# zakuro-ai/asr

Measured on AMD Instinct MI355X. Metric: utterances/sec (10 s, 161-bin) DS2 5x1024 BiGRU CTC train step, higher is better.
Workload: dtype bf16

## Files before the change

### asr_amd/csrc/conv_bf16.hip

```cpp
#include "common.h"
#include <stdlib.h>

namespace {

typedef __bf16 bf16x8 __attribute__((ext_vector_type(8)));

constexpr int TT = 128, KT = 11, PT = 5, CH = 32;
constexpr int NPIX = TT + KT - 1;
constexpr int IPITCH = 80;
constexpr int WROW = KT * 2 * 2 * 32 * 16;

__device__ __attribute__((aligned(16))) float g_zero_cb[4] = {0.f, 0.f, 0.f, 0.f};

struct CArgs {
  const __bf16* in;
  const __bf16* wpk;
  const float* bias;
  float* out;
  const int* lens;
  int B, Din, T, Dtot, KD, SD, PD, OS, OO;
  int gx, gy, gz;
};

constexpr int IN_CHUNKS = NPIX * 4;
constexpr int IN_IT = (IN_CHUNKS + 255) / 256;
constexpr int W_CHUNKS = WROW / 16;
constexpr int W_IT = (W_CHUNKS + 255) / 256;

template <int SD, int R>
__global__ __launch_bounds__(256) void conv2_bf16_rows_kernel(CArgs a, int n_out, float* __restrict__ stat_part) {
  constexpr int RING = (R - 1) * SD + 1;
  constexpr int SLOT = NPIX * IPITCH;
  __shared__ __attribute__((aligned(16))) char in_lds[RING * SLOT];
  __shared__ __attribute__((aligned(16))) char w_lds[WROW];
  const int tid = threadIdx.x, lane = tid & 63, wave = tid >> 6;
  const int half = lane >> 5, l31 = lane & 31;
  int bx, by, bz;
  {
    const int total = a.gx * a.gy * a.gz, id = blockIdx.x;
    const int lin = (total & 7) == 0 ? (id & 7) * (total >> 3) + (id >> 3) : id;
    by = lin % a.gy;
    const int pair = lin / a.gy;
    bx = pair % a.gx; bz = pair / a.gx;
  }
  const int t0 = bx * TT, o0 = R * by, b = bz;
  const int len = a.lens ? min(a.lens[b], a.T) : a.T;
  const int t = t0 + wave * 32 + l31;
  auto out_ptr = [&](int o, int co) { return a.out + (((long long)b * CH + co) * a.Dtot + (a.OS * o + a.OO)) * a.T + t; };
  if (t0 >= len) {
    if (t < a.T) {
#pragma unroll
      for (int q = 0; q < R; ++q)
        if (o0 + q < n_out) {
#pragma unroll
          for (int r = 0; r < 16; ++r) *out_ptr(o0 + q, (r & 3) + 8 * (r >> 2) + 4 * half) = 0.f;
        }
    }
    return;
  }
  f32x16 acc[R];
#pragma unroll
  for (int q = 0; q < R; ++q)
#pragma unroll
    for (int r = 0; r < 16; ++r) acc[q][r] = 0.f;

  const int f0 = SD * o0 - a.PD;
  f32x4 ri[IN_IT], rw[W_IT];
  auto load_in = [&](int f) {
    const bool rowok = f >= 0 && f < a.Din;
    const char* rowp = reinterpret_cast<const char*>(a.in + (((long long)b * a.Din + (rowok ? f : 0)) * a.T) * CH);
#pragma unroll
    for (int u = 0; u < IN_IT; ++u) {
      const int c = tid + 256 * u;
      const int pix = c >> 2, q = c & 3;
      const int tt = t0 - PT + pix;
      const bool ok = rowok && c < IN_CHUNKS && tt >= 0 && tt < a.T;
      const void* p = ok ? (const void*)(rowp + ((long long)tt * CH) * 2 + q * 16) : (const void*)g_zero_cb;
      ri[u] = *reinterpret_cast<const f32x4*>(p);
    }
  };
  auto store_in = [&](int slot) {
#pragma unroll
    for (int u = 0; u < IN_IT; ++u) {
      const int c = tid + 256 * u;
      if (c < IN_CHUNKS) *reinterpret_cast<f32x4*>(in_lds + slot * SLOT + (c >> 2) * IPITCH + (c & 3) * 16) = ri[u];
    }
  };
  auto load_w = [&](int kd) {
    const char* wp = reinterpret_cast<const char*>(a.wpk) + (long long)kd * WROW;
#pragma unroll
    for (int u = 0; u < W_IT; ++u) {
      const int c = tid + 256 * u;
      rw[u] = *reinterpret_cast<const f32x4*>(wp + (c < W_CHUNKS ? c : 0) * 16);
    }
  };
  auto store_w = [&]() {
#pragma unroll
    for (int u = 0; u < W_IT; ++u) {
      const int c = tid + 256 * u;
      if (c < W_CHUNKS) *reinterpret_cast<f32x4*>(w_lds + c * 16) = rw[u];
    }
  };
#pragma unroll
  for (int j = 0; j < RING - 1; ++j) {
    load_in(f0 + j);
    store_in(j);
  }
  load_in(f0 + RING - 1);
  load_w(0);
  const int pix_off = (wave * 32 + l31) * IPITCH + half * 16;
  const char* abase = w_lds + half * (32 * 16) + l31 * 16;
  int slot0 = 0;
  for (int kd = 0; kd < a.KD; ++kd) {
    __syncthreads();
    {
      int snew = slot0 + RING - 1;
      if (snew >= RING) snew -= RING;
      store_in(snew);
    }
    store_w();
    __syncthreads();
    if (kd + 1 < a.KD) {
      load_in(f0 + kd + RING);
      load_w(kd + 1);
    }
    const char* bq[R];
#pragma unroll
    for (int q = 0; q < R; ++q) {
      int sl = slot0 + q * SD;
      if (sl >= RING) sl -= RING;
      bq[q] = in_lds + sl * SLOT + pix_off;
    }
#pragma unroll
    for (int kt = 0; kt < KT; ++kt) {
#pragma unroll
      for (int kk = 0; kk < 2; ++kk) {
        const bf16x8 af = *reinterpret_cast<const bf16x8*>(abase + (kt * 2 + kk) * (2 * 32 * 16));
#pragma unroll
        for (int q = 0; q < R; ++q) {
          const bf16x8 x = *reinterpret_cast<const bf16x8*>(bq[q] + kt * IPITCH + kk * 32);
          acc[q] = __builtin_amdgcn_mfma_f32_32x32x16_bf16(af, x, acc[q], 0, 0, 0);
        }
      }
    }
    slot0 = slot0 + 1 == RING ? 0 : slot0 + 1;
  }
  float bv[16];
#pragma unroll
  for (int r = 0; r < 16; ++r) bv[r] = a.bias ? a.bias[(r & 3) + 8 * (r >> 2) + 4 * half] : 0.f;
  float s1[16], s2[16];
#pragma unroll
  for (int r = 0; r < 16; ++r) { s1[r] = 0.f; s2[r] = 0.f; }
#pragma unroll
  for (int q = 0; q < R; ++q)
    if (o0 + q < n_out) {
#pragma unroll
      for (int r = 0; r < 16; ++r) {
        const float v = (t >= len || t >= a.T) ? 0.f : acc[q][r] + bv[r];
        if (t < a.T) *out_ptr(o0 + q, (r & 3) + 8 * (r >> 2) + 4 * half) = v;
        s1[r] += v;
        s2[r] += v * v;
      }
    }
  if (stat_part) {
    __shared__ float red[4][32][2];
#pragma unroll
    for (int r = 0; r < 16; ++r) {
#pragma unroll
      for (int m = 1; m < 32; m <<= 1) { s1[r] += __shfl_xor(s1[r], m); s2[r] += __shfl_xor(s2[r], m); }
      if (l31 == 0) { const int co = (r & 3) + 8 * (r >> 2) + 4 * half; red[wave][co][0] = s1[r]; red[wave][co][1] = s2[r]; }
    }
    __syncthreads();
    if (tid < 64) {
      const int co = tid >> 1, w = tid & 1;
      const float sum = ((red[0][co][w] + red[1][co][w]) + red[2][co][w]) + red[3][co][w];
      const long long blk = ((long long)bz * a.gy + by) * a.gx + bx;
      stat_part[(blk * 32 + co) * 2 + w] = sum;
    }
  }
}

__global__ __launch_bounds__(256) void nhwc_cast_kernel(const float* __restrict__ src, __bf16* __restrict__ dst, int Bn, int D, int T) {
  __shared__ float tile[CH][65];
  const int t0 = blockIdx.x * 64, d = blockIdx.y, b = blockIdx.z;
  const int tx = threadIdx.x & 63, ty = threadIdx.x >> 6;
#pragma unroll
  for (int i = 0; i < 8; ++i) {
    const int c = ty + 4 * i, t = t0 + tx;
    tile[c][tx] = (t < T) ? src[(((long long)b * CH + c) * D + d) * T + t] : 0.f;
  }
  __syncthreads();
  const int c = threadIdx.x & 31, tq = threadIdx.x >> 5;
#pragma unroll
  for (int i = 0; i < 8; ++i) {
    const int tl = tq + 8 * i, t = t0 + tl;
    if (t < T) dst[(((long long)b * D + d) * T + t) * CH + c] = (__bf16)tile[c][tl];
  }
}

__global__ void pack_conv2_bf16_kernel(const float* __restrict__ W, __bf16* __restrict__ wf, __bf16* __restrict__ wd0, __bf16* __restrict__ wd1) {
  const int per_row = WROW / 2;
  const int nf = 21 * per_row, n0 = 11 * per_row, n1 = 10 * per_row;
  const int idx = blockIdx.x * blockDim.x + threadIdx.x;
  if (idx >= nf + n0 + n1) return;
  int which, i;
  if (idx < nf) { which = 0; i = idx; } else if (idx < nf + n0) { which = 1; i = idx - nf; } else { which = 2; i = idx - nf - n0; }
  const int j = i & 7, m = (i >> 3) & 31, kg = (i >> 8) & 1, kk = (i >> 9) & 1;
  const int rest = i >> 10;
  const int kt = rest % KT, kdr = rest / KT;
  const int kch = kk * 16 + kg * 8 + j;
  float v;
  if (which == 0) {
    v = W[((m * 32 + kch) * 21 + kdr) * 11 + kt];
    wf[i] = (__bf16)v;
  } else {
    const int p = which - 1, KDe = (21 - p + 1) / 2;
    v = W[((kch * 32 + m) * 21 + (2 * (KDe - 1 - kdr) + p)) * 11 + (10 - kt)];
    (which == 1 ? wd0 : wd1)[i] = (__bf16)v;
  }
}

}

extern "C" size_t ds2_conv2_bf16_packed_bytes(int which) { return (size_t)(which == 0 ? 21 : which == 1 ? 11 : 10) * WROW; }

extern "C" int ds2_conv2_pack_bf16(const float* w2, void* wf, void* wd0, void* wd1, void* stream) {
  DS2_REQUIRE(w2 && wf && wd0 && wd1, "ds2_conv2_pack_bf16: null pointer");
  const int total = (21 + 11 + 10) * (WROW / 2);
  hipLaunchKernelGGL(pack_conv2_bf16_kernel, dim3(ceil_div(total, 256)), dim3(256), 0, (hipStream_t)stream, w2, (__bf16*)wf, (__bf16*)wd0,
                     (__bf16*)wd1);
  DS2_LAUNCH_CHECK("pack_conv2_bf16_kernel");
  return 0;
}

extern "C" int ds2_nhwc_bf16_f32(const float* src, void* dst, int B, int D, int T, void* stream) {
  DS2_REQUIRE(src && dst && B > 0 && D > 0 && T > 0, "ds2_nhwc_bf16_f32: bad args");
  hipLaunchKernelGGL(nhwc_cast_kernel, dim3(ceil_div(T, 64), D, B), dim3(256), 0, (hipStream_t)stream, src, (__bf16*)dst, B, D, T);
  DS2_LAUNCH_CHECK("nhwc_cast_kernel");
  return 0;
}

extern "C" int ds2_conv2_fwd_bf16_stat_blocks(int B, int D1, int T) {
  const int D2 = (D1 + 2 * 10 - 21) / 2 + 1;
  return ceil_div(T, TT) * ceil_div(D2, 3) * B;
}

extern "C" int ds2_conv2_fwd_bf16_stats(const void* a1_nhwc, const void* wf, const float* bias, const int* lens_dev, float* y2, int B, int D1,
                                        int T, float* stat_part, void* stream) {
  DS2_REQUIRE(a1_nhwc && wf && y2, "ds2_conv2_fwd_bf16: null pointer");
  const int D2 = (D1 + 2 * 10 - 21) / 2 + 1;
  CArgs a{};
  a.in = (const __bf16*)a1_nhwc; a.wpk = (const __bf16*)wf; a.bias = bias; a.out = y2; a.lens = lens_dev;
  a.B = B; a.Din = D1; a.T = T; a.Dtot = D2; a.KD = 21; a.SD = 2; a.PD = 10; a.OS = 1; a.OO = 0;
  if (stat_part) DS2_HIP(hipMemsetAsync(stat_part, 0, (size_t)ds2_conv2_fwd_bf16_stat_blocks(B, D1, T) * 64 * sizeof(float), (hipStream_t)stream));
  a.gx = ceil_div(T, TT); a.gy = ceil_div(D2, 3); a.gz = B;
  hipLaunchKernelGGL((conv2_bf16_rows_kernel<2, 3>), dim3(a.gx * a.gy * a.gz), dim3(256), 0, (hipStream_t)stream, a, D2, stat_part);
  DS2_LAUNCH_CHECK("conv2_bf16_rows_kernel fwd");
  return 0;
}

extern "C" int ds2_conv2_fwd_bf16(const void* a1_nhwc, const void* wf, const float* bias, const int* lens_dev, float* y2, int B, int D1,
                                  int T, void* stream) {
  return ds2_conv2_fwd_bf16_stats(a1_nhwc, wf, bias, lens_dev, y2, B, D1, T, nullptr, stream);
}

extern "C" int ds2_conv2_dgrad_bf16(const void* dy2_nhwc, const void* wd0, const void* wd1, float* da1, int B, int D1, int T, void* stream) {
  DS2_REQUIRE(dy2_nhwc && wd0 && wd1 && da1, "ds2_conv2_dgrad_bf16: null pointer");
  const int D2 = (D1 + 2 * 10 - 21) / 2 + 1;
  for (int p = 0; p < 2; ++p) {
    const int KDe = (21 - p + 1) / 2;
    const int n_o = (D1 - p + 1) / 2;
    CArgs a{};
    a.in = (const __bf16*)dy2_nhwc; a.wpk = (const __bf16*)(p == 0 ? wd0 : wd1); a.bias = nullptr; a.out = da1; a.lens = nullptr;
    a.B = B; a.Din = D2; a.T = T; a.Dtot = D1; a.KD = KDe; a.SD = 1; a.PD = KDe - 6; a.OS = 2; a.OO = p;
    a.gx = ceil_div(T, TT); a.gy = ceil_div(n_o, 4); a.gz = B;
    hipLaunchKernelGGL((conv2_bf16_rows_kernel<1, 4>), dim3(a.gx * a.gy * a.gz), dim3(256), 0, (hipStream_t)stream, a, n_o, (float*)nullptr);
  }
  DS2_LAUNCH_CHECK("conv2_bf16_rows_kernel dgrad");
  return 0;
}

namespace {

constexpr int WT = 64;
constexpr int WK = WT + 16;
constexpr int WPITCH = 176;
constexpr int KDG = 3;
constexpr int TAPS = KDG * KT;
constexpr int TPW = (TAPS + 3) / 4;

struct WArgs {
  const __bf16* a1p;
  const __bf16* dyp;
  float* part;
  const int* lens;
  int B, D1, D2, T, Tp, pairs_per_chunk;
};

typedef unsigned int u32x4 __attribute__((ext_vector_type(4)));

__device__ __forceinline__ void store_shifted_copies(const u32x4 lo, const u32x4 hi, char* dst ) {
  const unsigned W[8] = {lo.x, lo.y, lo.z, lo.w, hi.x, hi.y, hi.z, hi.w};
#pragma unroll
  for (int r = 0; r < 8; ++r) {
    const int w0 = (8 - r) >> 1;
    u32x4 o;
    if ((r & 1) == 0) {
      o = u32x4{W[w0], W[w0 + 1], W[w0 + 2], W[w0 + 3]};
    } else {
      o = u32x4{__builtin_amdgcn_alignbit(W[w0 + 1], W[w0], 16), __builtin_amdgcn_alignbit(W[w0 + 2], W[w0 + 1], 16),
                __builtin_amdgcn_alignbit(W[w0 + 3], W[w0 + 2], 16), __builtin_amdgcn_alignbit(W[w0 + 4], W[w0 + 3], 16)};
    }
    *reinterpret_cast<u32x4*>(dst + r * 32 * WPITCH) = o;
  }
}

__global__ __launch_bounds__(256) __attribute__((amdgpu_waves_per_eu(2, 2))) void conv2_wgrad_bf16_kernel(WArgs a) {
  __shared__ __attribute__((aligned(16))) char dy_lds[8 * 32 * WPITCH];
  __shared__ __attribute__((aligned(16))) char a1_lds[KDG * 32 * WPITCH];
  const int tid = threadIdx.x, lane = tid & 63;
  const int wave = __builtin_amdgcn_readfirstlane(tid >> 6);
  const int l31 = lane & 31, half = lane >> 5;
  const int grp = blockIdx.x, chunk = blockIdx.y;
  const int kd0 = grp * KDG;

  f32x16 acc[TPW];
#pragma unroll
  for (int i = 0; i < TPW; ++i)
#pragma unroll
    for (int r = 0; r < 16; ++r) acc[i][r] = 0.f;

  constexpr int NDY = 2, NA1 = (KDG * 32 * 10 + 255) / 256;
  u32x4 dlo[NDY], dhi[NDY], av[NA1];

  const int npairs = a.B * a.D2;
  const int pend = min(npairs, (chunk + 1) * a.pairs_per_chunk);
  int p = chunk * a.pairs_per_chunk, t0 = 0, len = 0;
  auto settle = [&]() {
    while (p < pend) {
      len = a.lens ? min(a.lens[p / a.D2], a.T) : a.T;
      if (t0 < len) return true;
      ++p;
      t0 = 0;
    }
    return false;
  };
  auto load_tile = [&]() {
    const int b = p / a.D2, o = p % a.D2;
#pragma unroll
    for (int k = 0; k < NDY; ++k) {
      const int idx = tid + 256 * k;
      const int co = idx / 11, m = idx % 11;
      const __bf16* row = a.dyp + (((long long)b * 32 + min(co, 31)) * a.D2 + o) * a.Tp;
      const int xl = t0 - 8 + m * 8, xh = xl + 8;
      const bool okl = idx < 352 && m >= 2 && m < 2 + WT / 8 && xl + 8 <= a.Tp;
      const bool okh = idx < 352 && m + 1 >= 2 && m + 1 < 2 + WT / 8 && xh + 8 <= a.Tp;
      dlo[k] = *reinterpret_cast<const u32x4*>(okl ? (const void*)(row + xl) : (const void*)g_zero_cb);
      dhi[k] = *reinterpret_cast<const u32x4*>(okh ? (const void*)(row + xh) : (const void*)g_zero_cb);
    }
#pragma unroll
    for (int k = 0; k < NA1; ++k) {
      const int c = tid + 256 * k;
      const int ch = c % 10, ci = (c / 10) % 32, kdl = c / 320;
      const int f = 2 * o + (kd0 + kdl) - 10;
      const int x0 = t0 + ch * 8;
      const bool ok = c < KDG * 320 && (kd0 + kdl) < 21 && f >= 0 && f < a.D1 && x0 + 8 <= a.Tp;
      av[k] = *reinterpret_cast<const u32x4*>(ok ? (const void*)(a.a1p + (((long long)b * 32 + ci) * a.D1 + f) * a.Tp + x0)
                                                 : (const void*)g_zero_cb);
    }
  };

  bool have = settle();
  if (have) load_tile();
  while (have) {
    __syncthreads();
#pragma unroll
    for (int k = 0; k < NDY; ++k) {
      const int idx = tid + 256 * k;
      if (idx < 352) store_shifted_copies(dlo[k], dhi[k], dy_lds + (idx / 11) * WPITCH + (idx % 11) * 16);
    }
#pragma unroll
    for (int k = 0; k < NA1; ++k) {
      const int c = tid + 256 * k;
      if (c < KDG * 320) *reinterpret_cast<u32x4*>(a1_lds + ((c / 320) * 32 + (c / 10) % 32) * WPITCH + (c % 10) * 16) = av[k];
    }
    __syncthreads();
    t0 += WT;
    have = settle();
    if (have) load_tile();
    const char* ap[3];
#pragma unroll
    for (int q = 0; q < 3; ++q) {
      const int kt = min(wave + 4 * q, KT - 1);
      const int s = kt - PT;
      const int r = s & 7;
      const int joff = (s < 0) ? 8 : 0;
      ap[q] = dy_lds + (r * 32 + l31) * WPITCH + (8 * half + joff) * 2;
    }
    const char* bp = a1_lds + l31 * WPITCH + (8 * half) * 2;
#pragma unroll
    for (int ks = 0; ks < WK / 16; ++ks) {
      bf16x8 af[3], bfr[KDG];
#pragma unroll
      for (int q = 0; q < 3; ++q) af[q] = *reinterpret_cast<const bf16x8*>(ap[q] + ks * 32);
#pragma unroll
      for (int kdl = 0; kdl < KDG; ++kdl) bfr[kdl] = *reinterpret_cast<const bf16x8*>(bp + kdl * 32 * WPITCH + ks * 32);
#pragma unroll
      for (int q = 0; q < 3; ++q)
#pragma unroll
        for (int kdl = 0; kdl < KDG; ++kdl) acc[q * KDG + kdl] = __builtin_amdgcn_mfma_f32_32x32x16_bf16(af[q], bfr[kdl], acc[q * KDG + kdl], 0, 0, 0);
    }
  }
#pragma unroll
  for (int i = 0; i < TPW; ++i) {
    const int kt = wave + 4 * (i / KDG), kdl = i % KDG;
    if (kt < KT) {
      const int tap = kdl * KT + kt;
      float* out = a.part + ((((long long)chunk * gridDim.x + grp) * TAPS + tap) * 32) * 32;
#pragma unroll
      for (int r = 0; r < 16; ++r) {
        const int co = (r & 3) + 8 * (r >> 2) + 4 * half;
        out[co * 32 + l31] = acc[i][r];
      }
    }
  }
}

__global__ void conv2_wgrad_bf16_reduce_kernel(const float* __restrict__ part, float* __restrict__ dW, int chunks, int ngroups) {
  const int j = blockIdx.x * blockDim.x + threadIdx.x;
  const int per_chunk = ngroups * TAPS * 32 * 32;
  if (j >= per_chunk) return;
  const int ci = j & 31, co = (j >> 5) & 31, tap = (j >> 10) % TAPS, grp = (j >> 10) / TAPS;
  const int kd = grp * KDG + tap / KT, kt = tap % KT;
  float s = 0.f;
  int c = 0;
  for (; c + 8 <= chunks; c += 8) {
    float v[8];
#pragma unroll
    for (int k = 0; k < 8; ++k) v[k] = part[(long long)(c + k) * per_chunk + j];
#pragma unroll
    for (int k = 0; k < 8; ++k) s += v[k];
  }
  for (; c < chunks; ++c) s += part[(long long)c * per_chunk + j];
  if (kd < 21) dW[((co * 32 + ci) * 21 + kd) * 11 + kt] = s;
}

__global__ __launch_bounds__(256) void padcast_kernel(const float* __restrict__ src, __bf16* __restrict__ dst, long long R, int T, int Tp) {
  const int cq = Tp / 8;
  const long long total = R * cq;
  for (long long i = (long long)blockIdx.x * blockDim.x + threadIdx.x; i < total; i += (long long)gridDim.x * blockDim.x) {
    const long long r = i / cq;
    const int x0 = (int)(i % cq) * 8;
    bf16x8 o;
#pragma unroll
    for (int e = 0; e < 8; ++e) {
      const int t = x0 + e - 8;
      o[e] = (__bf16)((t >= 0 && t < T) ? src[r * T + t] : 0.f);
    }
    *reinterpret_cast<bf16x8*>(dst + r * Tp + x0) = o;
  }
}

}


namespace {
constexpr int NS = 128;
constexpr int NA1 = NS + 16;
constexpr int SEG_DY = NS * 64;
constexpr int SEG_A1 = NA1 * 64;
constexpr int SEG_BYTES = SEG_DY + KDG * SEG_A1;
typedef __attribute__((address_space(3))) void lds_void_c;
typedef const __attribute__((address_space(1))) void gbl_void_c;
typedef float f32x2c __attribute__((ext_vector_type(2)));

struct W2Args {
  const __bf16* a1n;
  const __bf16* dyn;
  float* part;
  const int* lens;
  int B, D1, D2, T, pairs_per_chunk, nchunks, chunks_per_xcd;
};

__global__ __launch_bounds__(256) __attribute__((amdgpu_waves_per_eu(2, 2))) void conv2_wgrad_nhwc_kernel(W2Args a) {
  extern __shared__ __attribute__((aligned(1024))) char seg[];
  const int tid = threadIdx.x, lane = tid & 63;
  const int wave = __builtin_amdgcn_readfirstlane(tid >> 6);
  const int l31 = lane & 31, half = lane >> 5;
  const int xcd = blockIdx.x & 7, slot = blockIdx.x >> 3;
  const int chunk = xcd * a.chunks_per_xcd + slot / 7, grp = slot % 7;
  if (slot >= 7 * a.chunks_per_xcd || chunk >= a.nchunks) return;
  const int kd0 = grp * KDG;

  f32x16 acc[TPW];
#pragma unroll
  for (int i = 0; i < TPW; ++i)
#pragma unroll
    for (int r = 0; r < 16; ++r) acc[i][r] = 0.f;

  const int npairs = a.B * a.D2;
  const int pbeg = chunk * a.pairs_per_chunk, pend = min(npairs, pbeg + a.pairs_per_chunk);
  int p = pbeg, t0 = 0;
  auto settle = [&]() {
    while (t0 < a.T) {
      while (p < pend) {
        const int len = a.lens ? min(a.lens[p / a.D2], a.T) : a.T;
        if (t0 < len) return true;
        ++p;
      }
      p = pbeg;
      t0 += NS;
    }
    return false;
  };
  const int prow = lane >> 2, pq = (lane & 3) * 8;
  auto stage = [&](int buf, int sp, int st0) {
    const int b = sp / a.D2, o = sp % a.D2;
    char* base = seg + buf * SEG_BYTES;
    const __bf16* dyrow = a.dyn + ((long long)(b * a.D2 + o) * a.T) * 32;
#pragma unroll
    for (int i = 0; i < 2; ++i) {
      const int piece = wave + 4 * i;
      const int t = st0 + piece * 16 + prow;
      const void* src = t < a.T ? (const void*)(dyrow + (long long)t * 32 + pq) : (const void*)g_zero_cb;
      __builtin_amdgcn_global_load_lds((gbl_void_c*)src, (lds_void_c*)(base + piece * 1024), 16, 0, 0);
    }
#pragma unroll
    for (int i = 0; i < 7; ++i) {
      const int idx = wave + 4 * i;
      if (idx < KDG * 9) {
        const int kdl = idx / 9, piece = idx % 9;
        const int f = 2 * o + (kd0 + kdl) - 10;
        const int t = st0 - 8 + piece * 16 + prow;
        const bool ok = (kd0 + kdl) < 21 && f >= 0 && f < a.D1 && t >= 0 && t < a.T;
        const void* src = ok ? (const void*)(a.a1n + ((long long)(b * a.D1 + f) * a.T + t) * 32 + pq) : (const void*)g_zero_cb;
        __builtin_amdgcn_global_load_lds((gbl_void_c*)src, (lds_void_c*)(base + SEG_DY + kdl * SEG_A1 + piece * 1024), 16, 0, 0);
      }
    }
  };

  const unsigned lds0 = (unsigned)(uintptr_t)(lds_void_c*)seg;
  const int p16 = lane & 15, g16 = (lane >> 4) & 1;
  const unsigned lanepart = (unsigned)((half * 8 + (p16 >> 2)) * 64 + (g16 * 16 + 4 * (p16 & 3)) * 2);
  const unsigned dyaddr = lds0 + lanepart;
  unsigned a1addr[3];
#pragma unroll
  for (int q = 0; q < 3; ++q) {
    const int kt = min(wave + 4 * q, KT - 1);
    a1addr[q] = lds0 + SEG_DY + (unsigned)((kt - PT + 8) * 64) + lanepart;
  }

  bool have = settle();
  int cur = 0;
  int np = p, nt0 = t0;
  if (have) stage(0, p, t0);
  while (have) {
    nt0 = t0; np = p + 1;
    { const int sp = p, st = t0; p = np; t0 = nt0; const bool more = settle(); np = p; nt0 = t0; p = sp; t0 = st; have = more; }
    asm volatile("s_waitcnt vmcnt(0)" ::: "memory");
    __syncthreads();
    if (have) stage(cur ^ 1, np, nt0);
    const unsigned boff = (unsigned)(cur * SEG_BYTES);
    f32x4 fd[2], fg[2][KDG];
#define W2_RD(dst, addr, off)                                                                                                         \
    do {                                                                                                                              \
      f32x2c lo_, hi_;                                                                                                                \
      asm volatile("ds_read_b64_tr_b16 %0, %2 offset:%3\n\tds_read_b64_tr_b16 %1, %2 offset:%4"                                        \
                   : "=&v"(lo_), "=&v"(hi_)                                                                                           \
                   : "v"(addr), "n"(off), "n"((off) + 256));                                                                          \
      dst = __builtin_shufflevector(lo_, hi_, 0, 1, 2, 3);                                                                            \
    } while (0)
#define W2_GROUP_RD(slot, ks, q)                                                                                                      \
    do {                                                                                                                              \
      W2_RD(fg[slot][0], a1addr[q] + boff, (ks) * 1024);                                                                              \
      W2_RD(fg[slot][1], a1addr[q] + boff, (ks) * 1024 + SEG_A1);                                                                     \
      W2_RD(fg[slot][2], a1addr[q] + boff, (ks) * 1024 + 2 * SEG_A1);                                                                 \
    } while (0)
#define W2_GROUP_MMA(slot, dslot, q, NWAIT)                                                                                           \
    do {                                                                                                                              \
      asm volatile("s_waitcnt lgkmcnt(%4)" : "+v"(fd[dslot]), "+v"(fg[slot][0]), "+v"(fg[slot][1]), "+v"(fg[slot][2]) : "n"(NWAIT) : "memory"); \
      _Pragma("unroll") for (int kdl = 0; kdl < KDG; ++kdl)                                                                           \
        acc[(q) * KDG + kdl] = __builtin_amdgcn_mfma_f32_32x32x16_bf16(__builtin_bit_cast(bf16x8, fd[dslot]), __builtin_bit_cast(bf16x8, fg[slot][kdl]), \
                                                                      acc[(q) * KDG + kdl], 0, 0, 0);                                  \
      __builtin_amdgcn_sched_barrier(0);                                                                                              \
    } while (0)
    W2_RD(fd[0], dyaddr + boff, 0);
    W2_GROUP_RD(0, 0, 0);
#pragma unroll
    for (int ks = 0; ks < NS / 16; ++ks) {
      const int s0 = (3 * ks) & 1, d = ks & 1;
      W2_GROUP_RD(s0 ^ 1, ks, 1);
      __builtin_amdgcn_sched_barrier(0);
      W2_GROUP_MMA(s0, d, 0, 6);
      W2_GROUP_RD(s0, ks, 2);
      __builtin_amdgcn_sched_barrier(0);
      W2_GROUP_MMA(s0 ^ 1, d, 1, 6);
      if (ks + 1 < NS / 16) {
        W2_RD(fd[d ^ 1], dyaddr + boff, (ks + 1) * 1024);
        W2_GROUP_RD(s0 ^ 1, ks + 1, 0);
        __builtin_amdgcn_sched_barrier(0);
        W2_GROUP_MMA(s0, d, 2, 8);
      } else {
        W2_GROUP_MMA(s0, d, 2, 0);
      }
    }
#undef W2_RD
#undef W2_GROUP_RD
#undef W2_GROUP_MMA
    p = np; t0 = nt0; cur ^= 1;
  }
#pragma unroll
  for (int i = 0; i < TPW; ++i) {
    const int kt = wave + 4 * (i / KDG), kdl = i % KDG;
    if (kt < KT) {
      const int tap = kdl * KT + kt;
      float* out = a.part + ((((long long)chunk * 7 + grp) * TAPS + tap) * 32) * 32;
#pragma unroll
      for (int r = 0; r < 16; ++r) {
        const int co = (r & 3) + 8 * (r >> 2) + 4 * half;
        out[co * 32 + l31] = acc[i][r];
      }
    }
  }
}
}

extern "C" int ds2_conv_padded_pitch(int T) { return (T + 16 + 7) / 8 * 8; }

extern "C" int ds2_padcast_bf16(const float* src, void* dst, long long R, int T, void* stream) {
  DS2_REQUIRE(src && dst && R > 0 && T > 0, "ds2_padcast_bf16: bad args");
  const int Tp = ds2_conv_padded_pitch(T);
  long long blocks = (R * (Tp / 8) + 255) / 256;
  if (blocks > 16384) blocks = 16384;
  hipLaunchKernelGGL(padcast_kernel, dim3((unsigned)blocks), dim3(256), 0, (hipStream_t)stream, src, (__bf16*)dst, R, T, Tp);
  DS2_LAUNCH_CHECK("padcast_kernel");
  return 0;
}

extern "C" size_t ds2_conv2_wgrad_bf16_workspace_bytes(int B, int D1) {
  const int D2 = (D1 + 2 * 10 - 21) / 2 + 1;
  const int pairs = B * D2;
  const int chunks = pairs < 73 ? pairs : 73;
  return (size_t)chunks * 7 * TAPS * 32 * 32 * sizeof(float);
}

extern "C" int ds2_conv2_wgrad_bf16(const void* a1p, const void* dy2p, const int* lens_dev, float* dW2, int B, int D1, int T, void* ws,
                                    size_t ws_bytes, void* stream) {
  DS2_REQUIRE(a1p && dy2p && dW2 && ws, "ds2_conv2_wgrad_bf16: null pointer");
  DS2_REQUIRE(ws_bytes >= ds2_conv2_wgrad_bf16_workspace_bytes(B, D1), "ds2_conv2_wgrad_bf16: workspace too small");
  const int D2 = (D1 + 2 * 10 - 21) / 2 + 1;
  const int pairs = B * D2;
  int chunks = pairs < 73 ? pairs : 73;
  const int ppc = ceil_div(pairs, chunks);
  chunks = ceil_div(pairs, ppc);
  WArgs a{};
  a.a1p = (const __bf16*)a1p; a.dyp = (const __bf16*)dy2p; a.part = (float*)ws; a.lens = lens_dev;
  a.B = B; a.D1 = D1; a.D2 = D2; a.T = T; a.Tp = ds2_conv_padded_pitch(T); a.pairs_per_chunk = ppc;
  hipStream_t s = (hipStream_t)stream;
  hipLaunchKernelGGL(conv2_wgrad_bf16_kernel, dim3(7, chunks), dim3(256), 0, s, a);
  DS2_LAUNCH_CHECK("conv2_wgrad_bf16_kernel");
  hipLaunchKernelGGL(conv2_wgrad_bf16_reduce_kernel, dim3(ceil_div(7 * TAPS * 32 * 32, 256)), dim3(256), 0, s, (const float*)ws, dW2, chunks, 7);
  DS2_LAUNCH_CHECK("conv2_wgrad_bf16_reduce_kernel");
  return 0;
}

extern "C" int ds2_conv2_wgrad_nhwc_bf16(const void* a1_nhwc, const void* dy2_nhwc, const int* lens_dev, float* dW2, int B, int D1, int T, void* ws,
                                         size_t ws_bytes, void* stream) {
  DS2_REQUIRE(a1_nhwc && dy2_nhwc && dW2 && ws, "ds2_conv2_wgrad_nhwc_bf16: null pointer");
  DS2_REQUIRE(ws_bytes >= ds2_conv2_wgrad_bf16_workspace_bytes(B, D1), "ds2_conv2_wgrad_nhwc_bf16: workspace too small");
  const int D2 = (D1 + 2 * 10 - 21) / 2 + 1;
  const int pairs = B * D2;
  constexpr int CPX = 9;
  int chunks = pairs < 8 * CPX ? pairs : 8 * CPX;
  const int ppc = ceil_div(pairs, chunks);
  chunks = ceil_div(pairs, ppc);
  W2Args a{};
  a.a1n = (const __bf16*)a1_nhwc; a.dyn = (const __bf16*)dy2_nhwc; a.part = (float*)ws; a.lens = lens_dev;
  a.B = B; a.D1 = D1; a.D2 = D2; a.T = T; a.pairs_per_chunk = ppc; a.nchunks = chunks; a.chunks_per_xcd = ceil_div(chunks, 8);
  hipStream_t s = (hipStream_t)stream;
  static bool attr = false;
  if (!attr) {
    DS2_HIP(hipFuncSetAttribute((const void*)conv2_wgrad_nhwc_kernel, hipFuncAttributeMaxDynamicSharedMemorySize, 2 * SEG_BYTES));
    attr = true;
  }
  hipLaunchKernelGGL(conv2_wgrad_nhwc_kernel, dim3(8 * (7 * a.chunks_per_xcd + 1)), dim3(256), 2 * SEG_BYTES, s, a);
  DS2_LAUNCH_CHECK("conv2_wgrad_nhwc_kernel");
  hipLaunchKernelGGL(conv2_wgrad_bf16_reduce_kernel, dim3(ceil_div(7 * TAPS * 32 * 32, 256)), dim3(256), 0, s, (const float*)ws, dW2, chunks, 7);
  DS2_LAUNCH_CHECK("conv2_wgrad_bf16_reduce_kernel");
  return 0;
}
```

Before: 2832.

## Rewrite conv2 rows kernel with async LDS DMA, 16x16 MFMA and merged dgrad launch

The conv2 forward/dgrad row kernel now stages input rows and weights with global_load_lds straight into LDS. It uses an extra ring slot and double-buffered weights so the next depth step's copy overlaps the current MFMA loop. It switches from 32x32x16 to 16x16x32 MFMA with software-pipelined hand-written ds_read_b128 and explicit lgkmcnt waits. It also uses a swizzled LDS layout, 8-wave blocks with larger time tiles and vectorized float4 output stores. The two dgrad parity launches are merged into one grid, and the weight packing is changed to match the new fragment layout. This adds inline asm and a larger dynamic LDS footprint, which may reduce occupancy.

Result: no change. 2851, median of 6 (+0.7%).

```diff
diff --git a/asr_amd/csrc/conv_bf16.hip b/asr_amd/csrc/conv_bf16.hip
--- a/asr_amd/csrc/conv_bf16.hip
+++ b/asr_amd/csrc/conv_bf16.hip
@@ -1,40 +1,79 @@
 #include "common.h"
 #include <stdlib.h>
+#include <stdint.h>
 
 namespace {
 
 typedef __bf16 bf16x8 __attribute__((ext_vector_type(8)));
-
-constexpr int TT = 128, KT = 11, PT = 5, CH = 32;
-constexpr int NPIX = TT + KT - 1;
-constexpr int IPITCH = 80;
-constexpr int WROW = KT * 2 * 2 * 32 * 16;
+typedef float f32x4u __attribute__((ext_vector_type(4), aligned(4)));
+typedef __attribute__((address_space(3))) void lds_void_c;
+typedef const __attribute__((address_space(1))) void gbl_void_c;
+
+constexpr int KT = 11, PT = 5, CH = 32;
+constexpr int WROW = KT * 2 * 64 * 16;
+constexpr int WPIECES = WROW / 1024;
 
 __device__ __attribute__((aligned(16))) float g_zero_cb[4] = {0.f, 0.f, 0.f, 0.f};
+
+struct CSet {
+  const __bf16* wpk;
+  int KD, PD, OO, n_out;
+};
 
 struct CArgs {
   const __bf16* in;
-  const __bf16* wpk;
   const float* bias;
   float* out;
   const int* lens;
-  int B, Din, T, Dtot, KD, SD, PD, OS, OO;
+  CSet s[2];
+  int B, Din, T, Dtot, OS;
   int gx, gy, gz;
+  int gy0;
 };
 
-constexpr int IN_CHUNKS = NPIX * 4;
-constexpr int IN_IT = (IN_CHUNKS + 255) / 256;
-constexpr int W_CHUNKS = WROW / 16;
-constexpr int W_IT = (W_CHUNKS + 255) / 256;
-
-template <int SD, int R>
-__global__ __launch_bounds__(256) void conv2_bf16_rows_kernel(CArgs a, int n_out, float* __restrict__ stat_part) {
-  constexpr int RING = (R - 1) * SD + 1;
-  constexpr int SLOT = NPIX * IPITCH;
-  __shared__ __attribute__((aligned(16))) char in_lds[RING * SLOT];
-  __shared__ __attribute__((aligned(16))) char w_lds[WROW];
-  const int tid = threadIdx.x, lane = tid & 63, wave = tid >> 6;
-  const int half = lane >> 5, l31 = lane & 31;
+template <int SD, int R, int NW>
+struct RowsCfg {
+  static constexpr int TTB = NW * 32;
+  static constexpr int NPC = (TTB + KT - 1 + 15) / 16;
+  static constexpr int SLOT = NPC * 1024;
+  static constexpr int RING = (R - 1) * SD + 1;
+  static constexpr int NSLOT = RING + 1;
+  static constexpr int LDS = NSLOT * SLOT + 2 * WROW;
+};
+
+#define C2_RD(dst, addr, off) asm volatile("ds_read_b128 %0, %1 offset:%2" : "=v"(dst) : "v"(addr), "n"(off))
+#define C2_RDG(s_, kt_, q_)                                                                                                          \
+  do {                                                                                                                                \
+    if ((q_) == 0) {                                                                                                                  \
+      C2_RD(af[s_][0], wa, ((kt_) * 2) * 1024);                                                                                       \
+      C2_RD(af[s_][1], wa, ((kt_) * 2 + 1) * 1024);                                                                                   \
+    }                                                                                                                                 \
+    const unsigned xa_ = rowb[q_] + (unsigned)poff[kt_];                                                                              \
+    C2_RD(xf[s_][q_][0], xa_, 0);                                                                                                     \
+    C2_RD(xf[s_][q_][1], xa_, 1024);                                                                                                  \
+  } while (0)
+#define C2_MMA(s_, q_, NWAIT_)                                                                                                        \
+  do {                                                                                                                                \
+    if ((q_) == 0)                                                                                                                    \
+      asm volatile("s_waitcnt lgkmcnt(%4)" : "+v"(af[s_][0]), "+v"(af[s_][1]), "+v"(xf[s_][0][0]), "+v"(xf[s_][0][1]) : "n"(NWAIT_) : "memory"); \
+    else                                                                                                                              \
+      asm volatile("s_waitcnt lgkmcnt(%2)" : "+v"(xf[s_][q_][0]), "+v"(xf[s_][q_][1]) : "n"(NWAIT_) : "memory");                       \
+    _Pragma("unroll") for (int h_ = 0; h_ < 2; ++h_)                                                                                  \
+      _Pragma("unroll") for (int c_ = 0; c_ < 2; ++c_)                                                                                \
+        acc[q_][h_][c_] = __builtin_amdgcn_mfma_f32_16x16x32_bf16(__builtin_bit_cast(bf16x8, xf[s_][q_][h_]),                         \
+                                                                  __builtin_bit_cast(bf16x8, af[s_][c_]), acc[q_][h_][c_], 0, 0, 0);  \
+    __builtin_amdgcn_sched_barrier(0);                                                                                                \
+  } while (0)
+
+template <int SD, int R, int NW>
+__global__ __launch_bounds__(NW * 64) void conv2_bf16_rows_kernel(CArgs a, float* __restrict__ stat_part) {
+  using Cfg = RowsCfg<SD, R, NW>;
+  constexpr int TTB = Cfg::TTB, NPC = Cfg::NPC, SLOT = Cfg::SLOT, RING = Cfg::RING, NSLOT = Cfg::NSLOT;
+  extern __shared__ __attribute__((aligned(1024))) char lds[];
+  char* const w_lds = lds + NSLOT * SLOT;
+  const int tid = threadIdx.x, lane = tid & 63;
+  const int wave = __builtin_amdgcn_readfirstlane(tid >> 6);
+  const int l15 = lane & 15, seg = lane >> 4;
   int bx, by, bz;
   {
     const int total = a.gx * a.gy * a.gz, id = blockIdx.x;
@@ -43,142 +82,167 @@
     const int pair = lin / a.gy;
     bx = pair % a.gx; bz = pair / a.gx;
   }
-  const int t0 = bx * TT, o0 = R * by, b = bz;
+  const int cls = by >= a.gy0 ? 1 : 0;
+  const CSet cs = a.s[cls];
+  const int t0 = bx * TTB, o0 = R * (by - (cls ? a.gy0 : 0)), b = bz;
   const int len = a.lens ? min(a.lens[b], a.T) : a.T;
-  const int t = t0 + wave * 32 + l31;
-  auto out_ptr = [&](int o, int co) { return a.out + (((long long)b * CH + co) * a.Dtot + (a.OS * o + a.OO)) * a.T + t; };
+  const int n_out = cs.n_out;
+  const int tw = t0 + wave * 32 + 4 * seg;
+  auto store4 = [&](int o, int co, int t, const f32x4 v) {
+    float* p = a.out + (((long long)b * CH + co) * a.Dtot + (a.OS * o + cs.OO)) * a.T + t;
+    if (t + 3 < a.T) {
+      *reinterpret_cast<f32x4u*>(p) = v;
+    } else {
+#pragma unroll
+      for (int j = 0; j < 3; ++j)
+        if (t + j < a.T) p[j] = v[j];
+    }
+  };
   if (t0 >= len) {
-    if (t < a.T) {
-#pragma unroll
-      for (int q = 0; q < R; ++q)
-        if (o0 + q < n_out) {
-#pragma unroll
-          for (int r = 0; r < 16; ++r) *out_ptr(o0 + q, (r & 3) + 8 * (r >> 2) + 4 * half) = 0.f;
-        }
-    }
+#pragma unroll
+    for (int q = 0; q < R; ++q)
+      if (o0 + q < n_out) {
+#pragma unroll
+        for (int h = 0; h < 2; ++h)
+#pragma unroll
+          for (int c = 0; c < 2; ++c) store4(o0 + q, 16 * c + l15, tw + 16 * h, f32x4{0.f, 0.f, 0.f, 0.f});
+      }
     return;
   }
-  f32x16 acc[R];
+  f32x4 acc[R][2][2];
 #pragma unroll
   for (int q = 0; q < R; ++q)
 #pragma unroll
-    for (int r = 0; r < 16; ++r) acc[q][r] = 0.f;
-
-  const int f0 = SD * o0 - a.PD;
-  f32x4 ri[IN_IT], rw[W_IT];
-  auto load_in = [&](int f) {
+    for (int h = 0; h < 2; ++h)
+#pragma unroll
+      for (int c = 0; c < 2; ++c) acc[q][h][c] = f32x4{0.f, 0.f, 0.f, 0.f};
+
+  const int f0 = SD * o0 - cs.PD;
+  const int dpix = lane >> 2, dslot = lane & 3;
+  auto dma_row = [&](int f, int slot, int p) {
     const bool rowok = f >= 0 && f < a.Din;
-    const char* rowp = reinterpret_cast<const char*>(a.in + (((long long)b * a.Din + (rowok ? f : 0)) * a.T) * CH);
-#pragma unroll
-    for (int u = 0; u < IN_IT; ++u) {
-      const int c = tid + 256 * u;
-      const int pix = c >> 2, q = c & 3;
-      const int tt = t0 - PT + pix;
-      const bool ok = rowok && c < IN_CHUNKS && tt >= 0 && tt < a.T;
-      const void* p = ok ? (const void*)(rowp + ((long long)tt * CH) * 2 + q * 16) : (const void*)g_zero_cb;
-      ri[u] = *reinterpret_cast<const f32x4*>(p);
-    }
+    const int pix = p * 16 + dpix;
+    const int tt = t0 - PT + pix;
+    const int sg = dslot ^ (((pix >> 2) & 1) << 1);
+    const bool ok = rowok && tt >= 0 && tt < a.T;
+    const void* src = ok ? (const void*)(reinterpret_cast<const char*>(a.in) + ((((long long)b * a.Din + f) * a.T + tt) * CH) * 2 + sg * 16)
+                         : (const void*)g_zero_cb;
+    __builtin_amdgcn_global_load_lds((gbl_void_c*)src, (lds_void_c*)(lds + slot * SLOT + p * 1024), 16, 0, 0);
   };
-  auto store_in = [&](int slot) {
-#pragma unroll
-    for (int u = 0; u < IN_IT; ++u) {
-      const int c = tid + 256 * u;
-      if (c < IN_CHUNKS) *reinterpret_cast<f32x4*>(in_lds + slot * SLOT + (c >> 2) * IPITCH + (c & 3) * 16) = ri[u];
-    }
+  auto dma_w = [&](int kd, int p) {
+    const char* src = reinterpret_cast<const char*>(cs.wpk) + (long long)kd * WROW + p * 1024 + lane * 16;
+    __builtin_amdgcn_global_load_lds((gbl_void_c*)src, (lds_void_c*)(w_lds + (kd & 1) * WROW + p * 1024), 16, 0, 0);
   };
-  auto load_w = [&](int kd) {
-    const char* wp = reinterpret_cast<const char*>(a.wpk) + (long long)kd * WROW;
-#pragma unroll
-    for (int u = 0; u < W_IT; ++u) {
-      const int c = tid + 256 * u;
-      rw[u] = *reinterpret_cast<const f32x4*>(wp + (c < W_CHUNKS ? c : 0) * 16);
+  auto stage = [&](int f, int slot, int kd) {
+    constexpr int NIT = (NPC + WPIECES + NW - 1) / NW;
+#pragma unroll
+    for (int u = 0; u < NIT; ++u) {
+      const int i = wave + NW * u;
+      if (i < NPC) dma_row(f, slot, i);
+      else if (i < NPC + WPIECES) dma_w(kd, i - NPC);
     }
   };
-  auto store_w = [&]() {
-#pragma unroll
-    for (int u = 0; u < W_IT; ++u) {
-      const int c = tid + 256 * u;
-      if (c < W_CHUNKS) *reinterpret_cast<f32x4*>(w_lds + c * 16) = rw[u];
-    }
-  };
 #pragma unroll
   for (int j = 0; j < RING - 1; ++j) {
-    load_in(f0 + j);
-    store_in(j);
-  }
-  load_in(f0 + RING - 1);
-  load_w(0);
-  const int pix_off = (wave * 32 + l31) * IPITCH + half * 16;
-  const char* abase = w_lds + half * (32 * 16) + l31 * 16;
+    constexpr int NIT = (NPC + NW - 1) / NW;
+#pragma unroll
+    for (int u = 0; u < NIT; ++u) {
+      const int i = wave + NW * u;
+      if (i < NPC) dma_row(f0 + j, j, i);
+    }
+  }
+  stage(f0 + RING - 1, RING - 1, 0);
+
+  int poff[KT];
+#pragma unroll
+  for (int kt = 0; kt < KT; ++kt) {
+    const int p = wave * 32 + l15 + kt;
+    poff[kt] = p * 64 + ((seg ^ (((p >> 2) & 1) << 1)) << 4);
+  }
+  const unsigned lds0 = (unsigned)(uintptr_t)(lds_void_c*)lds;
   int slot0 = 0;
-  for (int kd = 0; kd < a.KD; ++kd) {
+  for (int kd = 0; kd < cs.KD; ++kd) {
+    asm volatile("s_waitcnt vmcnt(0)" ::: "memory");
     __syncthreads();
-    {
-      int snew = slot0 + RING - 1;
-      if (snew >= RING) snew -= RING;
-      store_in(snew);
-    }
-    store_w();
-    __syncthreads();
-    if (kd + 1 < a.KD) {
-      load_in(f0 + kd + RING);
-      load_w(kd + 1);
-    }
-    const char* bq[R];
+    unsigned rowb[R];
 #pragma unroll
     for (int q = 0; q < R; ++q) {
       int sl = slot0 + q * SD;
-      if (sl >= RING) sl -= RING;
-      bq[q] = in_lds + sl * SLOT + pix_off;
-    }
+      if (sl >= NSLOT) sl -= NSLOT;
+      rowb[q] = lds0 + (unsigned)(sl * SLOT);
+    }
+    const unsigned wa = lds0 + (unsigned)(NSLOT * SLOT + (kd & 1) * WROW + lane * 16);
+    f32x4 af[2][2], xf[2][R][2];
+#pragma unroll
+    for (int q = 0; q < R; ++q) C2_RDG(0, 0, q);
+    __builtin_amdgcn_sched_barrier(0);
+    if (kd + 1 < cs.KD) {
+      int snew = slot0 + RING;
+      if (snew >= NSLOT) snew -= NSLOT;
+      stage(f0 + kd + RING, snew, kd + 1);
+    }
+    __builtin_amdgcn_sched_barrier(0);
 #pragma unroll
     for (int kt = 0; kt < KT; ++kt) {
-#pragma unroll
-      for (int kk = 0; kk < 2; ++kk) {
-        const bf16x8 af = *reinterpret_cast<const bf16x8*>(abase + (kt * 2 + kk) * (2 * 32 * 16));
-#pragma unroll
-        for (int q = 0; q < R; ++q) {
-          const bf16x8 x = *reinterpret_cast<const bf16x8*>(bq[q] + kt * IPITCH + kk * 32);
-          acc[q] = __builtin_amdgcn_mfma_f32_32x32x16_bf16(af, x, acc[q], 0, 0, 0);
+      const int s = kt & 1;
+#pragma unroll
+      for (int q = 0; q < R; ++q) {
+        if (kt + 1 < KT) {
+          C2_RDG(s ^ 1, kt + 1, q);
+          __builtin_amdgcn_sched_barrier(0);
+          C2_MMA(s, q, 2 + 2 * R);
+        } else {
+          C2_MMA(s, q, 2 * (R - 1 - q));
         }
       }
     }
-    slot0 = slot0 + 1 == RING ? 0 : slot0 + 1;
-  }
-  float bv[16];
-#pragma unroll
-  for (int r = 0; r < 16; ++r) bv[r] = a.bias ? a.bias[(r & 3) + 8 * (r >> 2) + 4 * half] : 0.f;
-  float s1[16], s2[16];
-#pragma unroll
-  for (int r = 0; r < 16; ++r) { s1[r] = 0.f; s2[r] = 0.f; }
+    slot0 = slot0 + 1 == NSLOT ? 0 : slot0 + 1;
+  }
+  float bv[2];
+#pragma unroll
+  for (int c = 0; c < 2; ++c) bv[c] = a.bias ? a.bias[16 * c + l15] : 0.f;
+  float s1[2] = {0.f, 0.f}, s2[2] = {0.f, 0.f};
 #pragma unroll
   for (int q = 0; q < R; ++q)
     if (o0 + q < n_out) {
 #pragma unroll
-      for (int r = 0; r < 16; ++r) {
-        const float v = (t >= len || t >= a.T) ? 0.f : acc[q][r] + bv[r];
-        if (t < a.T) *out_ptr(o0 + q, (r & 3) + 8 * (r >> 2) + 4 * half) = v;
-        s1[r] += v;
-        s2[r] += v * v;
-      }
+      for (int h = 0; h < 2; ++h)
+#pragma unroll
+        for (int c = 0; c < 2; ++c) {
+          const int t = tw + 16 * h;
+          f32x4 v;
+#pragma unroll
+          for (int j = 0; j < 4; ++j) {
+            v[j] = (t + j >= len) ? 0.f : acc[q][h][c][j] + bv[c];
+            s1[c] += v[j];
+            s2[c] += v[j] * v[j];
+          }
+          store4(o0 + q, 16 * c + l15, t, v);
+        }
     }
   if (stat_part) {
-    __shared__ float red[4][32][2];
-#pragma unroll
-    for (int r = 0; r < 16; ++r) {
-#pragma unroll
-      for (int m = 1; m < 32; m <<= 1) { s1[r] += __shfl_xor(s1[r], m); s2[r] += __shfl_xor(s2[r], m); }
-      if (l31 == 0) { const int co = (r & 3) + 8 * (r >> 2) + 4 * half; red[wave][co][0] = s1[r]; red[wave][co][1] = s2[r]; }
+    float* red = reinterpret_cast<float*>(lds);
+    __syncthreads();
+#pragma unroll
+    for (int c = 0; c < 2; ++c) {
+      s1[c] += __shfl_xor(s1[c], 16); s2[c] += __shfl_xor(s2[c], 16);
+      s1[c] += __shfl_xor(s1[c], 32); s2[c] += __shfl_xor(s2[c], 32);
+      if (seg == 0) { red[(wave * 32 + 16 * c + l15) * 2] = s1[c]; red[(wave * 32 + 16 * c + l15) * 2 + 1] = s2[c]; }
     }
     __syncthreads();
     if (tid < 64) {
-      const int co = tid >> 1, w = tid & 1;
-      const float sum = ((red[0][co][w] + red[1][co][w]) + red[2][co][w]) + red[3][co][w];
+      float sum = red[tid];
+#pragma unroll
+      for (int w = 1; w < NW; ++w) sum += red[w * 64 + tid];
       const long long blk = ((long long)bz * a.gy + by) * a.gx + bx;
-      stat_part[(blk * 32 + co) * 2 + w] = sum;
-    }
-  }
-}
+      stat_part[blk * 64 + tid] = sum;
+    }
+  }
+}
+
+#undef C2_RD
+#undef C2_RDG
+#undef C2_MMA
 
 __global__ __launch_bounds__(256) void nhwc_cast_kernel(const float* __restrict__ src, __bf16* __restrict__ dst, int Bn, int D, int T) {
   __shared__ float tile[CH][65];
@@ -205,10 +269,9 @@
   if (idx >= nf + n0 + n1) return;
   int which, i;
   if (idx < nf) { which = 0; i = idx; } else if (idx < nf + n0) { which = 1; i = idx - nf; } else { which = 2; i = idx - nf - n0; }
-  const int j = i & 7, m = (i >> 3) & 31, kg = (i >> 8) & 1, kk = (i >> 9) & 1;
+  const int j = i & 7, m = ((i >> 9) & 1) * 16 + ((i >> 3) & 15), kch = ((i >> 7) & 3) * 8 + j;
   const int rest = i >> 10;
   const int kt = rest % KT, kdr = rest / KT;
-  const int kch = kk * 16 + kg * 8 + j;
   float v;
   if (which == 0) {
     v = W[((m * 32 + kch) * 21 + kdr) * 11 + kt];
@@ -220,6 +283,20 @@
   }
 }
 
+constexpr int FWD_R = 3, FWD_NW = 8, DG_R = 4, DG_NW = 8;
+
+template <int SD, int R, int NW>
+int launch_rows(const CArgs& a, float* stat_part, hipStream_t s) {
+  using Cfg = RowsCfg<SD, R, NW>;
+  static bool attr = false;
+  if (!attr) {
+    DS2_HIP(hipFuncSetAttribute((const void*)conv2_bf16_rows_kernel<SD, R, NW>, hipFuncAttributeMaxDynamicSharedMemorySize, Cfg::LDS));
+    attr = true;
+  }
+  hipLaunchKernelGGL((conv2_bf16_rows_kernel<SD, R, NW>), dim3(a.gx * a.gy * a.gz), dim3(NW * 64), Cfg::LDS, s, a, stat_part);
+  return 0;
+}
+
 }
 
 extern "C" size_t ds2_conv2_bf16_packed_bytes(int which) { return (size_t)(which == 0 ? 21 : which == 1 ? 11 : 10) * WROW; }
@@ -242,19 +319,22 @@
 
 extern "C" int ds2_conv2_fwd_bf16_stat_blocks(int B, int D1, int T) {
   const int D2 = (D1 + 2 * 10 - 21) / 2 + 1;
-  return ceil_div(T, TT) * ceil_div(D2, 3) * B;
+  return ceil_div(T, RowsCfg<2, FWD_R, FWD_NW>::TTB) * ceil_div(D2, FWD_R) * B;
 }
 
 extern "C" int ds2_conv2_fwd_bf16_stats(const void* a1_nhwc, const void* wf, const float* bias, const int* lens_dev, float* y2, int B, int D1,
                                         int T, float* stat_part, void* stream) {
   DS2_REQUIRE(a1_nhwc && wf && y2, "ds2_conv2_fwd_bf16: null pointer");
+  DS2_REQUIRE(B > 0 && D1 > 0 && T > 0, "ds2_conv2_fwd_bf16: bad shape");
   const int D2 = (D1 + 2 * 10 - 21) / 2 + 1;
   CArgs a{};
-  a.in = (const __bf16*)a1_nhwc; a.wpk = (const __bf16*)wf; a.bias = bias; a.out = y2; a.lens = lens_dev;
-  a.B = B; a.Din = D1; a.T = T; a.Dtot = D2; a.KD = 21; a.SD = 2; a.PD = 10; a.OS = 1; a.OO = 0;
+  a.in = (const __bf16*)a1_nhwc; a.bias = bias; a.out = y2; a.lens = lens_dev;
+  a.s[0] = CSet{(const __bf16*)wf, 21, 10, 0, D2};
+  a.s[1] = a.s[0];
+  a.B = B; a.Din = D1; a.T = T; a.Dtot = D2; a.OS = 1;
   if (stat_part) DS2_HIP(hipMemsetAsync(stat_part, 0, (size_t)ds2_conv2_fwd_bf16_stat_blocks(B, D1, T) * 64 * sizeof(float), (hipStream_t)stream));
-  a.gx = ceil_div(T, TT); a.gy = ceil_div(D2, 3); a.gz = B;
-  hipLaunchKernelGGL((conv2_bf16_rows_kernel<2, 3>), dim3(a.gx * a.gy * a.gz), dim3(256), 0, (hipStream_t)stream, a, D2, stat_part);
+  a.gx = ceil_div(T, RowsCfg<2, FWD_R, FWD_NW>::TTB); a.gy = ceil_div(D2, FWD_R); a.gz = B; a.gy0 = a.gy;
+  if (launch_rows<2, FWD_R, FWD_NW>(a, stat_part, (hipStream_t)stream)) return 1;
   DS2_LAUNCH_CHECK("conv2_bf16_rows_kernel fwd");
   return 0;
 }
@@ -266,16 +346,20 @@
 
 extern "C" int ds2_conv2_dgrad_bf16(const void* dy2_nhwc, const void* wd0, const void* wd1, float* da1, int B, int D1, int T, void* stream) {
   DS2_REQUIRE(dy2_nhwc && wd0 && wd1 && da1, "ds2_conv2_dgrad_bf16: null pointer");
+  DS2_REQUIRE(B > 0 && D1 > 0 && T > 0, "ds2_conv2_dgrad_bf16: bad shape");
   const int D2 = (D1 + 2 * 10 - 21) / 2 + 1;
+  CArgs a{};
+  a.in = (const __bf16*)dy2_nhwc; a.bias = nullptr; a.out = da1; a.lens = nullptr;
+  int groups[2];
   for (int p = 0; p < 2; ++p) {
     const int KDe = (21 - p + 1) / 2;
     const int n_o = (D1 - p + 1) / 2;
-    CArgs a{};
-    a.in = (const __bf16*)dy2_nhwc; a.wpk = (const __bf16*)(p == 0 ? wd0 : wd1); a.bias = nullptr; a.out = da1; a.lens = nullptr;
-    a.B = B; a.Din = D2; a.T = T; a.Dtot = D1; a.KD = KDe; a.SD = 1; a.PD = KDe - 6; a.OS = 2; a.OO = p;
-    a.gx = ceil_div(T, TT); a.gy = ceil_div(n_o, 4); a.gz = B;
-    hipLaunchKernelGGL((conv2_bf16_rows_kernel<1, 4>), dim3(a.gx * a.gy * a.gz), dim3(256), 0, (hipStream_t)stream, a, n_o, (float*)nullptr);
-  }
+    a.s[p] = CSet{(const __bf16*)(p == 0 ? wd0 : wd1), KDe, KDe - 6, p, n_o};
+    groups[p] = ceil_div(n_o, DG_R);
+  }
+  a.B = B; a.Din = D2; a.T = T; a.Dtot = D1; a.OS = 2;
+  a.gx = ceil_div(T, RowsCfg<1, DG_R, DG_NW>::TTB); a.gy = groups[0] + groups[1]; a.gz = B; a.gy0 = groups[0];
+  if (launch_rows<1, DG_R, DG_NW>(a, nullptr, (hipStream_t)stream)) return 1;
   DS2_LAUNCH_CHECK("conv2_bf16_rows_kernel dgrad");
   return 0;
 }
@@ -470,8 +554,6 @@
 constexpr int SEG_DY = NS * 64;
 constexpr int SEG_A1 = NA1 * 64;
 constexpr int SEG_BYTES = SEG_DY + KDG * SEG_A1;
-typedef __attribute__((address_space(3))) void lds_void_c;
-typedef const __attribute__((address_space(1))) void gbl_void_c;
 typedef float f32x2c __attribute__((ext_vector_type(2)));
 
 struct W2Args {
```
